# CSMaus/DefectDetection_viaObjectDetection

Hardware: AMD Instinct MI355X
Metric: images/sec @640x640 b32 YOLOv8s-seg (higher is better)
Workload: dtype fp16

## Files before the change

defectdetection_viaobjectdetection_amd/csrc/conv_stem_c2.hip:

```cpp
#include <hip/hip_runtime.h>
#include <stdio.h>
#include <stdlib.h>

#include "common.h"
#include "switches.h"

namespace m355 {
namespace {

typedef float float16v __attribute__((ext_vector_type(16)));
typedef unsigned uint4v __attribute__((ext_vector_type(4)));

constexpr int TH = 8, TW = 16;
constexpr int PRR = 2 * TH + 1, PCC = 2 * TW + 1;
constexpr int PJ = 20;
constexpr int PATCH_BYTES = 43 * 1024;
constexpr int UR = 4 * TH + 3;
constexpr int UCH = 14;
constexpr int UP = 240;
constexpr int UDELTA = 7;
constexpr int U8_BYTES = UR * UP;
constexpr int NWAVES = 8;
constexpr int U8_OFF = 2 * PATCH_BYTES;
constexpr int BIAS_OFF = U8_OFF + 2 * U8_BYTES;
constexpr int W0_OFF = BIAS_OFF + 640;
constexpr int W2_OFF = W0_OFF + 2048;
constexpr int LDS_BYTES = W2_OFF + 8192;
constexpr int NPX = PRR * PCC;
static_assert((NPX + 15) / 16 == 36, "nine blocks of 16 patch pixels per wave of team X");

__device__ __forceinline__ void silu16(float16v& v) {
#pragma clang fp contract(off)
  float16v t;
#pragma unroll
  for (int j = 0; j < 16; ++j) t[j] = v[j] * -1.4426950408889634f;
#pragma unroll
  for (int j = 0; j < 16; ++j) t[j] = __builtin_amdgcn_exp2f(t[j]);
#pragma unroll
  for (int j = 0; j < 16; ++j) t[j] = 1.0f + t[j];
#pragma unroll
  for (int j = 0; j < 16; ++j) t[j] = __builtin_amdgcn_rcpf(t[j]);
#pragma unroll
  for (int j = 0; j < 16; ++j) v[j] = v[j] * t[j];
}

__global__ __launch_bounds__(512, 2) void stem_s2c32_cv1_v2_kernel(const ConvArgs a, const StemArgs st, int tiles_x, int tiles_y, int ntiles,
                                                                  int nxb) {
  extern __shared__ __attribute__((aligned(16))) char smem[];
  const int tid = threadIdx.x, lane = tid & 63;
  const int wave = __builtin_amdgcn_readfirstlane(tid >> 6);
  const int team = wave >> 2, wq = wave & 3;
  const int nwg = gridDim.x;
  const int IH = st.H, IW = st.W, rowb = IW * 3;

  if (tid < 64) ((float*)(smem + BIAS_OFF))[tid] = a.bias[tid];
  else if (tid < 128) ((float*)(smem + BIAS_OFF))[tid] = a.bias2[tid - 64];
  else if (tid < 160) ((float*)(smem + BIAS_OFF))[tid] = st.bias[tid - 128];
  if (tid >= 256 && tid < 256 + 128) {
    const int i = tid - 256, row = i >> 2, c = i & 3, mt = row >> 4, r = row & 15;
    const int chl = (r >> 2) * 8 + mt * 4 + (r & 3);
    *(float4v*)(smem + W0_OFF + row * 64 + c * 16) = *(const float4v*)(st.w16 + chl * 32 + c * 8);
  }

  auto decode = [&](int vb, int& tb, int& y0, int& x0) __attribute__((always_inline)) {
    const int xcd = vb & 7, q = ntiles >> 3, r = ntiles & 7;
    const int L = (nwg & 7) ? vb : (xcd < r ? xcd * (q + 1) : r * (q + 1) + (xcd - r) * q) + (vb >> 3);
    const int tx = L % tiles_x;
    const int rest = L / tiles_x;
    tb = rest / tiles_y;
    y0 = (rest - tb * tiles_y) * TH;
    x0 = tx * TW;
  };

  const __amdgpu_buffer_rsrc_t rs_in = __builtin_amdgcn_make_buffer_rsrc((void*)st.x, 0, st.B * IH * rowb, 0x00020000);
  uint4v u8v[2] = {{0u, 0u, 0u, 0u}, {0u, 0u, 0u, 0u}};
  auto window_load = [&](int tb, int y0, int x0) __attribute__((always_inline)) {
#pragma unroll
    for (int k = 0; k < 2; ++k) {
      const int t = (tid & 255) + 256 * k;
      const int ur = t / UCH, uc = t - ur * UCH;
      uint4v v = {0u, 0u, 0u, 0u};
      const int row = 4 * y0 - 3 + ur;
      const int cb = 12 * x0 - 9 - UDELTA + uc * 16;
      if (t < UR * UCH && (unsigned)row < (unsigned)IH) {
        v = __builtin_amdgcn_raw_buffer_load_b128(rs_in, (tb * IH + row) * rowb + cb, 0, 0);
        if (cb < 0 || cb + 16 > rowb) {
#pragma unroll
          for (int w = 0; w < 4; ++w) {
            unsigned m = 0;
#pragma unroll
            for (int j = 0; j < 4; ++j) {
              const int bi = cb + 4 * w + j;
              if (bi >= 0 && bi < rowb) m |= 0xffu << (8 * j);
            }
            v[w] &= m;
          }
        }
      }
      u8v[k] = v;
    }
  };
  auto window_store = [&](int buf) __attribute__((always_inline)) {
#pragma unroll
    for (int k = 0; k < 2; ++k) {
      const int t = (tid & 255) + 256 * k;
      const int ur = t / UCH, uc = t - ur * UCH;
      if (t < UR * UCH) *(uint4v*)(smem + U8_OFF + buf * U8_BYTES + ur * UP + uc * 16) = u8v[k];
    }
  };

  const int l15 = lane & 15, g = lane >> 4;
  auto stage_a = [&](int y0, int x0, int ubuf_i, int pbuf_i, int blk0, int nblk) __attribute__((always_inline)) {
    int toff[8];
#pragma unroll
    for (int j = 0; j < 8; ++j) {
      const int k = g * 8 + j;
      const int kh = k / 9, q = k - kh * 9;
      toff[j] = k < 27 ? kh * UP + q + UDELTA : UDELTA;
    }
    const unsigned char* const ubuf = (const unsigned char*)(smem + U8_OFF + ubuf_i * U8_BYTES);
    char* const pimg = smem + pbuf_i * PATCH_BYTES;
    const float inv255 = 1.0f / 255.0f;
    float b0[2][4];
#pragma unroll
    for (int mt = 0; mt < 2; ++mt) {
      const float4v u = *(const float4v*)(smem + BIAS_OFF + 512 + (8 * g + 4 * mt) * 4);
      b0[mt][0] = u[0]; b0[mt][1] = u[1]; b0[mt][2] = u[2]; b0[mt][3] = u[3];
    }
    auto gather = [&](int blk, int& dst, unsigned& keep) __attribute__((always_inline)) -> half8 {
      const int p = blk * 16 + l15;
      const bool pv = p < NPX;
      const int pp = pv ? p : NPX - 1;
      const int pr = pp / PCC, pc = pp - pr * PCC;
      const unsigned char* base = ubuf + (2 * pr) * UP + (2 * pc) * 3;
      half8 xf;
#pragma unroll
      for (int j = 0; j < 8; ++j) xf[j] = (half_t)(float)(unsigned)base[toff[j]];
      keep = ((y0 == 0 && pr == 0) || (x0 == 0 && pc == 0)) ? 0u : 0xffffffffu;
      const int jj = pc >> 1;
      const int R = pv ? (pr * 2 + (pc & 1)) * PJ + jj : PJ - 1;
      dst = R * 64 + ((g ^ ((jj >> 2) & 3)) << 4);
      return xf;
    };
    auto finish = [&](const float4v& acc0, const float4v& acc1, int dst, unsigned keep) __attribute__((always_inline)) {
      half8 o;
#pragma unroll
      for (int j = 0; j < 4; ++j) {
        o[j] = m355_to_half(m355_silu(acc0[j] * inv255 + b0[0][j]));
        o[4 + j] = m355_to_half(m355_silu(acc1[j] * inv255 + b0[1][j]));
      }
      uint4v ov = *(const uint4v*)&o;
      ov[0] &= keep; ov[1] &= keep; ov[2] &= keep; ov[3] &= keep;
      *(uint4v*)(pimg + dst) = ov;
    };
    const half8 wf0 = *(const half8*)(smem + W0_OFF + l15 * 64 + g * 16);
    const half8 wf1 = *(const half8*)(smem + W0_OFF + (16 + l15) * 64 + g * 16);
    const float4v z4 = {0.f, 0.f, 0.f, 0.f};
    for (int k = 0; k < nblk; ++k) {
      const int blk = blk0 + 4 * k;
      int d0;
      unsigned k0;
      const half8 x0f = gather(blk, d0, k0);
      const float4v a00 = __builtin_amdgcn_mfma_f32_16x16x32_f16(wf0, x0f, z4, 0, 0, 0);
      const float4v a01 = __builtin_amdgcn_mfma_f32_16x16x32_f16(wf1, x0f, z4, 0, 0, 0);
      finish(a00, a01, d0, k0);
    }
  };
  const int NXB = nxb;

  for (int i = tid; i < 8 * 64; i += 64 * NWAVES) *(float4v*)(smem + W2_OFF + i * 16) = *(const float4v*)(a.wf2 + (long)i * 8);
  half8 w1v[2][18];
  int tb_[3][2];
  const int h = lane >> 5, x15 = lane & 15, r2 = (lane >> 4) & 1;
  if (team == 1) {
#pragma unroll
    for (int b = 0; b < 2; ++b) {
      const half_t* wp = a.wf + (long)b * 18 * 512 + lane * 8;
#pragma unroll
      for (int s = 0; s < 18; ++s) w1v[b][s] = *(const half8*)(wp + 512 * s);
    }
#pragma unroll
    for (int kw = 0; kw < 3; ++kw) {
      const int j = x15 + (kw >> 1);
      const int row = ((2 * (2 * wq + r2)) * 2 + (kw & 1)) * PJ + j;
#pragma unroll
      for (int s = 0; s < 2; ++s) tb_[kw][s] = row * 64 + (((2 * s + h) ^ ((j >> 2) & 3)) << 4);
    }
  }
  auto stage_bc = [&](int tb, int y0, int x0, int pbuf_i) __attribute__((always_inline)) {
    const char* const pimg = smem + pbuf_i * PATCH_BYTES;
    float16v acc[2];
    {
      const float* bp = (const float*)(smem + BIAS_OFF) + 8 * h;
#pragma unroll
      for (int b = 0; b < 2; ++b)
#pragma unroll
        for (int s = 0; s < 2; ++s) {
          const float4v u0 = *(const float4v*)(bp + 32 * b + 16 * s), u1 = *(const float4v*)(bp + 32 * b + 16 * s + 4);
          acc[b][8 * s + 0] = u0[0]; acc[b][8 * s + 1] = u0[1]; acc[b][8 * s + 2] = u0[2]; acc[b][8 * s + 3] = u0[3];
          acc[b][8 * s + 4] = u1[0]; acc[b][8 * s + 5] = u1[1]; acc[b][8 * s + 6] = u1[2]; acc[b][8 * s + 7] = u1[3];
        }
    }
    half8 bf[2][2];
#pragma unroll
    for (int s = 0; s < 2; ++s) bf[0][s] = *(const half8*)(pimg + tb_[0][s]);
#pragma unroll
    for (int tap = 0; tap < 9; ++tap) {
      if (tap < 8) {
        const int nk = (tap + 1) / 3, nw = (tap + 1) - 3 * nk;
#pragma unroll
        for (int s = 0; s < 2; ++s) bf[(tap + 1) & 1][s] = *(const half8*)(pimg + tb_[nw][s] + nk * 2 * PJ * 64);
      }
#pragma unroll
      for (int s = 0; s < 2; ++s) {
        acc[0] = __builtin_amdgcn_mfma_f32_32x32x16_f16(w1v[0][tap * 2 + s], bf[tap & 1][s], acc[0], 0, 0, 0);
        acc[1] = __builtin_amdgcn_mfma_f32_32x32x16_f16(w1v[1][tap * 2 + s], bf[tap & 1][s], acc[1], 0, 0, 0);
      }
      __builtin_amdgcn_sched_barrier(0);
    }
    if (a.act) { silu16(acc[0]); silu16(acc[1]); }
    half8 zf[4];
#pragma unroll
    for (int b = 0; b < 2; ++b)
#pragma unroll
      for (int s = 0; s < 2; ++s)
#pragma unroll
        for (int j = 0; j < 8; ++j) zf[2 * b + s][j] = m355_to_half(acc[b][8 * s + j]);
    float16v acc2[2];
    {
      const float* bp = (const float*)(smem + BIAS_OFF) + 64 + 16 * h;
#pragma unroll
      for (int b = 0; b < 2; ++b)
#pragma unroll
        for (int qd = 0; qd < 4; ++qd) {
          const float4v u = *(const float4v*)(bp + 32 * b + 4 * qd);
          acc2[b][qd * 4 + 0] = u[0]; acc2[b][qd * 4 + 1] = u[1]; acc2[b][qd * 4 + 2] = u[2]; acc2[b][qd * 4 + 3] = u[3];
        }
    }
#pragma unroll
    for (int s = 0; s < 4; ++s) {
      const half8 wa = *(const half8*)(smem + W2_OFF + s * 1024 + lane * 16), wb = *(const half8*)(smem + W2_OFF + (4 + s) * 1024 + lane * 16);
      acc2[0] = __builtin_amdgcn_mfma_f32_32x32x16_f16(wa, zf[s], acc2[0], 0, 0, 0);
      acc2[1] = __builtin_amdgcn_mfma_f32_32x32x16_f16(wb, zf[s], acc2[1], 0, 0, 0);
    }
    silu16(acc2[0]);
    silu16(acc2[1]);
    const int yy = y0 + 2 * wq + r2, xx = x0 + x15;
    half_t* const yp = (half_t*)a.y + (long)tb * a.y_bstride + ((long)yy * a.Wo + xx) * a.ldy + 16 * h;
#pragma unroll
    for (int b = 0; b < 2; ++b)
#pragma unroll
      for (int half = 0; half < 2; ++half) {
        half8 o;
#pragma unroll
        for (int j = 0; j < 8; ++j) o[j] = m355_to_half(acc2[b][half * 8 + j]);
        *(half8*)(yp + 32 * b + half * 8) = o;
      }
  };

  int vb = blockIdx.x, tb, y0, x0;
  decode(vb, tb, y0, x0);
  if (team == 0) { window_load(tb, y0, x0); window_store(0); }
  __builtin_amdgcn_s_waitcnt(0x0070);
  __builtin_amdgcn_s_barrier();
  int nvb = vb + nwg < ntiles ? vb + nwg : -1;
  int ntb = 0, ny0 = 0, nx0 = 0;
  if (nvb >= 0) decode(nvb, ntb, ny0, nx0);
  if (team == 0) {
    if (nvb >= 0) window_load(ntb, ny0, nx0);
    stage_a(y0, x0, 0, 0, wq, NXB);
    if (nvb >= 0) window_store(1);
  } else {
    stage_a(y0, x0, 0, 0, wq + 4 * NXB, 9 - NXB);
  }
  asm volatile("s_waitcnt lgkmcnt(0)" ::: "memory");
  __builtin_amdgcn_s_barrier();

  for (int it = 0;; ++it) {
    const bool more = nvb >= 0;
    const int nnvb = more && nvb + nwg < ntiles ? nvb + nwg : -1;
    int nntb = 0, nny0 = 0, nnx0 = 0;
    if (nnvb >= 0) decode(nnvb, nntb, nny0, nnx0);
    if (team == 0) {
      if (more) {
        if (nnvb >= 0) window_load(nntb, nny0, nnx0);
        stage_a(ny0, nx0, (it + 1) & 1, (it + 1) & 1, wq, NXB);
        if (nnvb >= 0) window_store(it & 1);
      }
    } else {
      if (more) stage_a(ny0, nx0, (it + 1) & 1, (it + 1) & 1, wq + 4 * NXB, 9 - NXB);
      stage_bc(tb, y0, x0, it & 1);
    }
    if (!more) break;
    asm volatile("s_waitcnt lgkmcnt(0)" ::: "memory");
    __builtin_amdgcn_s_barrier();
    vb = nvb; nvb = nnvb;
    tb = ntb; y0 = ny0; x0 = nx0;
    ntb = nntb; ny0 = nny0; nx0 = nnx0;
  }
}

}

bool stem_s2c32_v2_ok(const ConvArgs& a, const StemArgs& st) {
  return stem_s2c32_ok(a, st) && a.wf && a.wf2;
}

int launch_stem_s2c32_v2(const ConvArgs& a, const StemArgs& st, hipStream_t s) {
  if (!stem_s2c32_v2_ok(a, st) || !conv_rows_covered(a, 64)) return -1;
  const int tiles_x = a.Wo / TW, tiles_y = a.Ho / TH;
  const int ntiles = st.B * tiles_y * tiles_x;
  static int slots = 0;
  if (!slots) {
    hipError_t e = hipFuncSetAttribute((const void*)stem_s2c32_cv1_v2_kernel, hipFuncAttributeMaxDynamicSharedMemorySize, LDS_BYTES);
    if (e != hipSuccess) return (int)e;
    int dev = 0, cus = 0;
    if (hipGetDevice(&dev) != hipSuccess || hipDeviceGetAttribute(&cus, hipDeviceAttributeMultiprocessorCount, dev) != hipSuccess)
      return -2;
    slots = cus & ~7;
    if (slots < 8) slots = 8;
  }
  const int grid = ntiles <= slots ? ntiles : slots;
  const int nxb_env = proc_switches().stem2_nxb;
  const int nxb = nxb_env < 5 ? 5 : (nxb_env > 9 ? 9 : nxb_env);
  hipLaunchKernelGGL(stem_s2c32_cv1_v2_kernel, dim3(grid), dim3(64 * NWAVES), LDS_BYTES, s, a, st, tiles_x, tiles_y, ntiles, nxb);
  return (int)hipGetLastError();
}

}
```

Baseline: 19080.

## Vectorize stem im2col gather with dword loads and software-pipeline stage A

Replaces the per-byte LDS gather of the uint8 input window with a few dword LDS loads that are realigned with alignbyte and packed into fp16 with cvt_pkrtz. For the producer team, stage A becomes a software pipeline that fetches two blocks ahead and issues the MFMA one block ahead of the SiLU/store epilogue. The main loop is also split into separate per-team loops so that the consumer team's weight registers and tap offsets exist only in that branch, which could lower register pressure. The intent is to cut LDS instruction count and hide LDS latency in the stem. The cost is more complex barrier pairing across the two teams and extra live registers in the pipelined path.

```diff
diff --git a/defectdetection_viaobjectdetection_amd/csrc/conv_stem_c2.hip b/defectdetection_viaobjectdetection_amd/csrc/conv_stem_c2.hip
--- a/defectdetection_viaobjectdetection_amd/csrc/conv_stem_c2.hip
+++ b/defectdetection_viaobjectdetection_amd/csrc/conv_stem_c2.hip
@@ -110,15 +110,20 @@
   };
 
   const int l15 = lane & 15, g = lane >> 4;
-  auto stage_a = [&](int y0, int x0, int ubuf_i, int pbuf_i, int blk0, int nblk) __attribute__((always_inline)) {
-    int toff[8];
-#pragma unroll
-    for (int j = 0; j < 8; ++j) {
-      const int k = g * 8 + j;
-      const int kh = k / 9, q = k - kh * 9;
-      toff[j] = k < 27 ? kh * UP + q + UDELTA : UDELTA;
-    }
-    const unsigned char* const ubuf = (const unsigned char*)(smem + U8_OFF + ubuf_i * U8_BYTES);
+  const int gk0 = 8 * g, gkh = gk0 / 9, gq = gk0 - 9 * gkh;
+  const bool two_runs = g == 1 || g == 2;
+  const int nA = two_runs ? 9 - gq : 0;
+  const int offA = g < 2 ? 8 : UP + 7;
+  const int offB = two_runs ? (gkh + 1) * UP - nA : gkh * UP + gq;
+  const unsigned maskA = (1u << (8 * nA)) - 1u;
+  struct ABlock {
+    unsigned a0, a1, b0, b1, b2;
+    int sha, shb;
+    int dst;
+    unsigned keep;
+  };
+  auto stage_a = [&](int y0, int x0, int ubuf_i, int pbuf_i, int blk0, int nblk, const bool pipe) __attribute__((always_inline)) {
+    const char* const ubuf = smem + U8_OFF + ubuf_i * U8_BYTES + UDELTA;
     char* const pimg = smem + pbuf_i * PATCH_BYTES;
     const float inv255 = 1.0f / 255.0f;
     float b0[2][4];
@@ -127,20 +132,34 @@
       const float4v u = *(const float4v*)(smem + BIAS_OFF + 512 + (8 * g + 4 * mt) * 4);
       b0[mt][0] = u[0]; b0[mt][1] = u[1]; b0[mt][2] = u[2]; b0[mt][3] = u[3];
     }
-    auto gather = [&](int blk, int& dst, unsigned& keep) __attribute__((always_inline)) -> half8 {
+    auto fetch = [&](int blk, ABlock& r) __attribute__((always_inline)) {
       const int p = blk * 16 + l15;
       const bool pv = p < NPX;
       const int pp = pv ? p : NPX - 1;
       const int pr = pp / PCC, pc = pp - pr * PCC;
-      const unsigned char* base = ubuf + (2 * pr) * UP + (2 * pc) * 3;
-      half8 xf;
-#pragma unroll
-      for (int j = 0; j < 8; ++j) xf[j] = (half_t)(float)(unsigned)base[toff[j]];
-      keep = ((y0 == 0 && pr == 0) || (x0 == 0 && pc == 0)) ? 0u : 0xffffffffu;
+      const int px = (2 * pr) * UP + (2 * pc) * 3;
+      const int sa = px + offA + UDELTA, sb = px + offB + UDELTA;
+      const unsigned* const pa = (const unsigned*)(ubuf + px + offA - (sa & 3));
+      const unsigned* const pb = (const unsigned*)(ubuf + px + offB - (sb & 3));
+      r.a0 = pa[0]; r.a1 = pa[1];
+      r.b0 = pb[0]; r.b1 = pb[1]; r.b2 = pb[2];
+      r.sha = sa & 3; r.shb = sb & 3;
+      r.keep = ((y0 == 0 && pr == 0) || (x0 == 0 && pc == 0)) ? 0u : 0xffffffffu;
       const int jj = pc >> 1;
       const int R = pv ? (pr * 2 + (pc & 1)) * PJ + jj : PJ - 1;
-      dst = R * 64 + ((g ^ ((jj >> 2) & 3)) << 4);
-      return xf;
+      r.dst = R * 64 + ((g ^ ((jj >> 2) & 3)) << 4);
+    };
+    auto operand = [&](const ABlock& r) __attribute__((always_inline)) -> half8 {
+      const unsigned ra = __builtin_amdgcn_alignbyte(r.a1, r.a0, r.sha);
+      const unsigned w0 = __builtin_amdgcn_alignbyte(r.b1, r.b0, r.shb), w1 = __builtin_amdgcn_alignbyte(r.b2, r.b1, r.shb);
+      const unsigned w[2] = {(ra & maskA) | (w0 & ~maskA), w1};
+      uint4v xv;
+#pragma unroll
+      for (int j = 0; j < 4; ++j) {
+        const unsigned u = w[j >> 1] >> (16 * (j & 1));
+        xv[j] = __builtin_bit_cast(unsigned, __builtin_amdgcn_cvt_pkrtz((float)(u & 0xffu), (float)((u >> 8) & 0xffu)));
+      }
+      return __builtin_bit_cast(half8, xv);
     };
     auto finish = [&](const float4v& acc0, const float4v& acc1, int dst, unsigned keep) __attribute__((always_inline)) {
       half8 o;
@@ -156,38 +175,42 @@
     const half8 wf0 = *(const half8*)(smem + W0_OFF + l15 * 64 + g * 16);
     const half8 wf1 = *(const half8*)(smem + W0_OFF + (16 + l15) * 64 + g * 16);
     const float4v z4 = {0.f, 0.f, 0.f, 0.f};
-    for (int k = 0; k < nblk; ++k) {
-      const int blk = blk0 + 4 * k;
-      int d0;
-      unsigned k0;
-      const half8 x0f = gather(blk, d0, k0);
-      const float4v a00 = __builtin_amdgcn_mfma_f32_16x16x32_f16(wf0, x0f, z4, 0, 0, 0);
-      const float4v a01 = __builtin_amdgcn_mfma_f32_16x16x32_f16(wf1, x0f, z4, 0, 0, 0);
-      finish(a00, a01, d0, k0);
-    }
-  };
-  const int NXB = nxb;
-
-  for (int i = tid; i < 8 * 64; i += 64 * NWAVES) *(float4v*)(smem + W2_OFF + i * 16) = *(const float4v*)(a.wf2 + (long)i * 8);
-  half8 w1v[2][18];
-  int tb_[3][2];
+    if (!pipe) {
+      for (int k = 0; k < nblk; ++k) {
+        ABlock r;
+        fetch(blk0 + 4 * k, r);
+        const half8 xf = operand(r);
+        const float4v a0 = __builtin_amdgcn_mfma_f32_16x16x32_f16(wf0, xf, z4, 0, 0, 0);
+        const float4v a1 = __builtin_amdgcn_mfma_f32_16x16x32_f16(wf1, xf, z4, 0, 0, 0);
+        finish(a0, a1, r.dst, r.keep);
+      }
+      return;
+    }
+    ABlock r[3];
+    float4v acc[2][2];
+    fetch(blk0, r[0]);
+    if (nblk > 1) fetch(blk0 + 4, r[1]);
+    {
+      const half8 xf = operand(r[0]);
+      acc[0][0] = __builtin_amdgcn_mfma_f32_16x16x32_f16(wf0, xf, z4, 0, 0, 0);
+      acc[0][1] = __builtin_amdgcn_mfma_f32_16x16x32_f16(wf1, xf, z4, 0, 0, 0);
+    }
+#pragma unroll
+    for (int k = 0; k < 9; ++k) {
+      if (k < nblk) {
+        if (k + 2 < nblk) fetch(blk0 + 4 * (k + 2), r[(k + 2) % 3]);
+        if (k + 1 < nblk) {
+          const half8 xf = operand(r[(k + 1) % 3]);
+          acc[(k + 1) & 1][0] = __builtin_amdgcn_mfma_f32_16x16x32_f16(wf0, xf, z4, 0, 0, 0);
+          acc[(k + 1) & 1][1] = __builtin_amdgcn_mfma_f32_16x16x32_f16(wf1, xf, z4, 0, 0, 0);
+        }
+        finish(acc[k & 1][0], acc[k & 1][1], r[k % 3].dst, r[k % 3].keep);
+      }
+    }
+  };
+
   const int h = lane >> 5, x15 = lane & 15, r2 = (lane >> 4) & 1;
-  if (team == 1) {
-#pragma unroll
-    for (int b = 0; b < 2; ++b) {
-      const half_t* wp = a.wf + (long)b * 18 * 512 + lane * 8;
-#pragma unroll
-      for (int s = 0; s < 18; ++s) w1v[b][s] = *(const half8*)(wp + 512 * s);
-    }
-#pragma unroll
-    for (int kw = 0; kw < 3; ++kw) {
-      const int j = x15 + (kw >> 1);
-      const int row = ((2 * (2 * wq + r2)) * 2 + (kw & 1)) * PJ + j;
-#pragma unroll
-      for (int s = 0; s < 2; ++s) tb_[kw][s] = row * 64 + (((2 * s + h) ^ ((j >> 2) & 3)) << 4);
-    }
-  }
-  auto stage_bc = [&](int tb, int y0, int x0, int pbuf_i) __attribute__((always_inline)) {
+  auto stage_bc = [&](const half8 (&w1v)[2][18], const int (&tb_)[3][2], int tb, int y0, int x0, int pbuf_i) __attribute__((always_inline)) {
     const char* const pimg = smem + pbuf_i * PATCH_BYTES;
     float16v acc[2];
     {
@@ -258,45 +281,71 @@
       }
   };
 
+  for (int i = tid; i < 8 * 64; i += 64 * NWAVES) *(float4v*)(smem + W2_OFF + i * 16) = *(const float4v*)(a.wf2 + (long)i * 8);
+
+  const int NXB = nxb;
+
   int vb = blockIdx.x, tb, y0, x0;
   decode(vb, tb, y0, x0);
-  if (team == 0) { window_load(tb, y0, x0); window_store(0); }
-  __builtin_amdgcn_s_waitcnt(0x0070);
-  __builtin_amdgcn_s_barrier();
   int nvb = vb + nwg < ntiles ? vb + nwg : -1;
   int ntb = 0, ny0 = 0, nx0 = 0;
   if (nvb >= 0) decode(nvb, ntb, ny0, nx0);
   if (team == 0) {
+    window_load(tb, y0, x0);
+    window_store(0);
+    __builtin_amdgcn_s_waitcnt(0x0070);
+    __builtin_amdgcn_s_barrier();
     if (nvb >= 0) window_load(ntb, ny0, nx0);
-    stage_a(y0, x0, 0, 0, wq, NXB);
+    stage_a(y0, x0, 0, 0, wq, NXB, true);
     if (nvb >= 0) window_store(1);
-  } else {
-    stage_a(y0, x0, 0, 0, wq + 4 * NXB, 9 - NXB);
-  }
-  asm volatile("s_waitcnt lgkmcnt(0)" ::: "memory");
-  __builtin_amdgcn_s_barrier();
-
-  for (int it = 0;; ++it) {
-    const bool more = nvb >= 0;
-    const int nnvb = more && nvb + nwg < ntiles ? nvb + nwg : -1;
-    int nntb = 0, nny0 = 0, nnx0 = 0;
-    if (nnvb >= 0) decode(nnvb, nntb, nny0, nnx0);
-    if (team == 0) {
-      if (more) {
-        if (nnvb >= 0) window_load(nntb, nny0, nnx0);
-        stage_a(ny0, nx0, (it + 1) & 1, (it + 1) & 1, wq, NXB);
-        if (nnvb >= 0) window_store(it & 1);
-      }
-    } else {
-      if (more) stage_a(ny0, nx0, (it + 1) & 1, (it + 1) & 1, wq + 4 * NXB, 9 - NXB);
-      stage_bc(tb, y0, x0, it & 1);
-    }
-    if (!more) break;
     asm volatile("s_waitcnt lgkmcnt(0)" ::: "memory");
     __builtin_amdgcn_s_barrier();
-    vb = nvb; nvb = nnvb;
-    tb = ntb; y0 = ny0; x0 = nx0;
-    ntb = nntb; ny0 = nny0; nx0 = nnx0;
+    for (int it = 0; nvb >= 0; ++it) {
+      const int nnvb = nvb + nwg < ntiles ? nvb + nwg : -1;
+      int nntb = 0, nny0 = 0, nnx0 = 0;
+      if (nnvb >= 0) {
+        decode(nnvb, nntb, nny0, nnx0);
+        window_load(nntb, nny0, nnx0);
+      }
+      stage_a(ny0, nx0, (it + 1) & 1, (it + 1) & 1, wq, NXB, true);
+      if (nnvb >= 0) window_store(it & 1);
+      asm volatile("s_waitcnt lgkmcnt(0)" ::: "memory");
+      __builtin_amdgcn_s_barrier();
+      nvb = nnvb;
+      ntb = nntb; ny0 = nny0; nx0 = nnx0;
+    }
+  } else {
+    half8 w1v[2][18];
+    int tb_[3][2];
+#pragma unroll
+    for (int b = 0; b < 2; ++b) {
+      const half_t* wp = a.wf + (long)b * 18 * 512 + lane * 8;
+#pragma unroll
+      for (int s = 0; s < 18; ++s) w1v[b][s] = *(const half8*)(wp + 512 * s);
+    }
+#pragma unroll
+    for (int kw = 0; kw < 3; ++kw) {
+      const int j = x15 + (kw >> 1);
+      const int row = ((2 * (2 * wq + r2)) * 2 + (kw & 1)) * PJ + j;
+#pragma unroll
+      for (int s = 0; s < 2; ++s) tb_[kw][s] = row * 64 + (((2 * s + h) ^ ((j >> 2) & 3)) << 4);
+    }
+    __builtin_amdgcn_s_waitcnt(0x0070);
+    __builtin_amdgcn_s_barrier();
+    stage_a(y0, x0, 0, 0, wq + 4 * NXB, 9 - NXB, false);
+    asm volatile("s_waitcnt lgkmcnt(0)" ::: "memory");
+    __builtin_amdgcn_s_barrier();
+    for (int it = 0;; ++it) {
+      const bool more = nvb >= 0;
+      if (more) stage_a(ny0, nx0, (it + 1) & 1, (it + 1) & 1, wq + 4 * NXB, 9 - NXB, false);
+      stage_bc(w1v, tb_, tb, y0, x0, it & 1);
+      if (!more) break;
+      asm volatile("s_waitcnt lgkmcnt(0)" ::: "memory");
+      __builtin_amdgcn_s_barrier();
+      tb = ntb; y0 = ny0; x0 = nx0;
+      nvb = nvb + nwg < ntiles ? nvb + nwg : -1;
+      if (nvb >= 0) decode(nvb, ntb, ny0, nx0);
+    }
   }
 }
 
```

Result: no change. 19070, median of 2 (-0.1%).
